# quadjr/aframe-gaussian-splatting

Hardware: AMD Instinct MI355X
Metric: frames/sec @1920x1080 (sort+project+bin+blend per frame, 1M-splat train.splat-shaped scene) (higher is better)
Workload: dtype f32

## Files before the change

### aframe-gaussian-splatting_amd/csrc/gs_prims.hip

```cpp
#include <type_traits>
#include "gs_internal.h"

namespace {

__device__ __forceinline__ uint32_t wave_incl_scan(uint32_t v, int lane)
{
#pragma unroll
    for (int d = 1; d < 64; d <<= 1) {
        const uint32_t t = __shfl_up(v, d, 64);
        if (lane >= d) v += t;
    }
    return v;
}

template <int NW>
__device__ __forceinline__ uint32_t block_excl_scan(uint32_t v, uint32_t *s_wave , uint32_t *total)
{
    const int lane = threadIdx.x & 63, w = threadIdx.x >> 6;
    const uint32_t inc = wave_incl_scan(v, lane);
    if (lane == 63) s_wave[w] = inc;
    __syncthreads();
    uint32_t base = 0, tot = 0;
#pragma unroll
    for (int k = 0; k < NW; k++) { const uint32_t s = s_wave[k]; if (k < w) base += s; tot += s; }
    __syncthreads();
    *total = tot;
    return base + inc - v;
}


template <bool PACKED, int NW>
__device__ __forceinline__ void k_radix_hist_body(const uint32_t *__restrict__ keys, const uint32_t *n_ptr, int shift,
                                                  int bits, uint32_t *__restrict__ hist)
{
    constexpr int NT = 64 * NW, IPT = 8, CH = NT * IPT;
    __shared__ uint32_t s_hist[GS_RADIX_MAX_BINS];
    const uint32_t n = *n_ptr;
    const uint32_t nchunks = (n + CH - 1) / CH;
    const uint32_t nbins = 1u << bits, mask = nbins - 1, rs = gs_radix_row_stride(nbins);
    for (uint32_t v = blockIdx.x; v < ((nchunks + 7u) & ~7u); v += gridDim.x) {
        uint32_t c;
        if (!gs_xcd_chunk(v, nchunks, c)) continue;
        for (uint32_t d = threadIdx.x; d < rs; d += NT) s_hist[d] = 0;
        __syncthreads();
        uint32_t kk[IPT];
#pragma unroll
        for (int r = 0; r < IPT; r++) {
            const uint32_t i = c * CH + r * NT + threadIdx.x;
            kk[r] = i < n ? keys[PACKED ? 2 * (size_t)i : i] : 0u;
        }
#pragma unroll
        for (int r = 0; r < IPT; r++) {
            const uint32_t i = c * CH + r * NT + threadIdx.x;
            if (i < n) atomicAdd(&s_hist[(kk[r] >> shift) & mask], 1u);
        }
        __syncthreads();
        for (uint32_t d = threadIdx.x; d < rs; d += NT) hist[(size_t)c * rs + d] = s_hist[d];
        __syncthreads();
    }
}

template <bool PACKED, int NW>
__global__ __launch_bounds__(64 * NW) void k_radix_hist(const uint32_t *__restrict__ keys, const uint32_t *n_ptr, int shift,
                                                        int bits, uint32_t *__restrict__ hist)
{
    k_radix_hist_body<PACKED, NW>(keys, n_ptr, shift, bits, hist);
}

template <int NW>
__device__ __forceinline__ void k_radix_scan_body(uint32_t *__restrict__ hist, const uint32_t *n_ptr, uint32_t chunk, int bits,
                                                  uint32_t *__restrict__ totals)
{
    constexpr int RC = 16;
    constexpr uint32_t LANES = 16u * NW;
    __shared__ uint4 s_part[NW][4];
    const uint32_t n = *n_ptr;
    const uint32_t nchunks = (n + chunk - 1) / chunk;
    const uint32_t nbins = 1u << bits, rs = gs_radix_row_stride(nbins);
    const uint32_t q = threadIdx.x & 3u, r = threadIdx.x >> 2;
    const int lane = threadIdx.x & 63, w = threadIdx.x >> 6;
    const uint32_t d0 = blockIdx.x * 16u + q * 4u;
    const bool dig_ok = d0 < rs;
    const uint32_t rpl = (nchunks + LANES - 1u) / LANES;
    const uint32_t c_lo = min(r * rpl, nchunks), c_hi = min(c_lo + rpl, nchunks);
    uint32_t *col = hist + d0;
    uint4 h[RC];
    uint4 run = make_uint4(0, 0, 0, 0);
#pragma unroll
    for (int k = 0; k < RC; k++) {
        h[k] = (dig_ok && c_lo + k < c_hi) ? *reinterpret_cast<const uint4 *>(col + (size_t)(c_lo + k) * rs) : make_uint4(0, 0, 0, 0);
    }
#pragma unroll
    for (int k = 0; k < RC; k++) { run.x += h[k].x; run.y += h[k].y; run.z += h[k].z; run.w += h[k].w; }
    if (dig_ok) {
        uint32_t c = c_lo + RC;
        for (; c + 8u <= c_hi; c += 8u) {
            uint4 t[8];
#pragma unroll
            for (int k = 0; k < 8; k++) t[k] = *reinterpret_cast<const uint4 *>(col + (size_t)(c + k) * rs);
#pragma unroll
            for (int k = 0; k < 8; k++) { run.x += t[k].x; run.y += t[k].y; run.z += t[k].z; run.w += t[k].w; }
        }
        for (; c < c_hi; c++) { const uint4 t = *reinterpret_cast<const uint4 *>(col + (size_t)c * rs); run.x += t.x; run.y += t.y; run.z += t.z; run.w += t.w; }
    }
    uint4 inc = run;
#pragma unroll
    for (int dlt = 4; dlt < 64; dlt <<= 1) {
        const uint32_t x = __shfl_up(inc.x, dlt, 64), y = __shfl_up(inc.y, dlt, 64), z = __shfl_up(inc.z, dlt, 64), ww = __shfl_up(inc.w, dlt, 64);
        if (lane >= dlt) { inc.x += x; inc.y += y; inc.z += z; inc.w += ww; }
    }
    if (lane >= 60) s_part[w][q] = inc;
    __syncthreads();
    uint4 base = make_uint4(inc.x - run.x, inc.y - run.y, inc.z - run.z, inc.w - run.w);
    uint4 grand = make_uint4(0, 0, 0, 0);
#pragma unroll
    for (int k = 0; k < NW; k++) {
        const uint4 p = s_part[k][q];
        if (k < w) { base.x += p.x; base.y += p.y; base.z += p.z; base.w += p.w; }
        grand.x += p.x; grand.y += p.y; grand.z += p.z; grand.w += p.w;
    }
    if (dig_ok) {
#pragma unroll
        for (int k = 0; k < RC; k++) {
            if (c_lo + k < c_hi) *reinterpret_cast<uint4 *>(col + (size_t)(c_lo + k) * rs) = base;
            base.x += h[k].x; base.y += h[k].y; base.z += h[k].z; base.w += h[k].w;
        }
        uint32_t c = c_lo + RC;
        for (; c + 8u <= c_hi; c += 8u) {
            uint4 t[8];
#pragma unroll
            for (int k = 0; k < 8; k++) t[k] = *reinterpret_cast<const uint4 *>(col + (size_t)(c + k) * rs);
#pragma unroll
            for (int k = 0; k < 8; k++) {
                *reinterpret_cast<uint4 *>(col + (size_t)(c + k) * rs) = base;
                base.x += t[k].x; base.y += t[k].y; base.z += t[k].z; base.w += t[k].w;
            }
        }
        for (; c < c_hi; c++) {
            const uint4 t = *reinterpret_cast<const uint4 *>(col + (size_t)c * rs);
            *reinterpret_cast<uint4 *>(col + (size_t)c * rs) = base;
            base.x += t.x; base.y += t.y; base.z += t.z; base.w += t.w;
        }
        if (r == 0) *reinterpret_cast<uint4 *>(totals + d0) = grand;
    }
}

template <int NW>
__global__ __launch_bounds__(64 * NW) void k_radix_scan(uint32_t *__restrict__ hist, const uint32_t *n_ptr, uint32_t chunk, int bits,
                                                        uint32_t *__restrict__ totals)
{
    k_radix_scan_body<NW>(hist, n_ptr, chunk, bits, totals);
}

template <int IN_FMT, int OUT_FMT, int MAXB, int NW>
__device__ __forceinline__ void k_radix_scatter_body(const void *__restrict__ in, void *__restrict__ out,
                                                     const uint32_t *n_ptr, int shift, int bits, uint32_t zero_key,
                                                     const uint32_t *__restrict__ hist_scanned, const uint32_t *__restrict__ totals,
                                                     int idx_bits, uint32_t *count_out, const uint32_t *fill_to)
{
    constexpr int NT = 64 * NW, IPT = 8, CH = NT * IPT;
    constexpr bool KEYONLY = (IN_FMT == GS_RADIX_KEYONLY && OUT_FMT == GS_RADIX_KEYONLY) || IN_FMT == GS_RADIX_KEYIDX;
    __shared__ uint32_t s_cnt[NW][MAXB];
    constexpr int MATCHB = MAXB <= 256 ? MAXB : 256;
    __shared__ unsigned long long s_match[NW][MATCHB];
    __shared__ uint32_t s_dbase[MAXB];
    __shared__ uint32_t s_gb[MAXB];
    __shared__ uint32_t s_k[CH];
    __shared__ uint32_t s_v[KEYONLY ? 1 : CH];
    __shared__ uint32_t s_wave[NW];
    const uint32_t n = *n_ptr;
    const uint32_t nchunks = (n + CH - 1) / CH;
    const uint32_t nbins = 1u << bits, mask = nbins - 1, rs = gs_radix_row_stride(nbins);
    const int lane = threadIdx.x & 63, w = threadIdx.x >> 6;
    const unsigned long long lt = (1ull << lane) - 1ull;
    if (IN_FMT == GS_RADIX_KEYIDX && fill_to) {
        const uint32_t upto = *fill_to;
        for (uint32_t i = n + blockIdx.x * NT + threadIdx.x; i < upto; i += gridDim.x * NT) reinterpret_cast<uint32_t *>(out)[i] = 0u;
    }
    if (blockIdx.x >= ((nchunks + 7u) & ~7u) && !(count_out && blockIdx.x == 0)) return;
    {
        constexpr int DPT = (MAXB + NT - 1) / NT;
        uint32_t tv[DPT], sum = 0;
#pragma unroll
        for (int k = 0; k < DPT; k++) { const uint32_t d = threadIdx.x * DPT + k; tv[k] = d < nbins ? totals[d] : 0u; sum += tv[k]; }
        uint32_t tot;
        uint32_t ex = block_excl_scan<NW>(sum, s_wave, &tot);
#pragma unroll
        for (int k = 0; k < DPT; k++) { const uint32_t d = threadIdx.x * DPT + k; if (d < nbins) s_dbase[d] = ex; ex += tv[k]; }
        if (count_out && blockIdx.x == 0 && threadIdx.x == 0) *count_out = tot;
    }
    for (uint32_t v = blockIdx.x; v < ((nchunks + 7u) & ~7u); v += gridDim.x) {
        uint32_t c;
        if (!gs_xcd_chunk(v, nchunks, c)) continue;
        for (uint32_t i = threadIdx.x; i < NW * MAXB; i += NT) { (&s_cnt[0][0])[i] = 0; if (i < NW * MATCHB) (&s_match[0][0])[i] = 0ull; }
        __syncthreads();
        uint32_t key[IPT], val[IPT], rank[IPT];
#pragma unroll
        for (int r = 0; r < IPT; r++) {
            const uint32_t i = c * CH + w * (CH / NW) + r * 64 + lane;
            const bool ok = i < n;
            if (IN_FMT == GS_RADIX_PACKED) {
                const uint2 kv = ok ? reinterpret_cast<const uint2 *>(in)[i] : make_uint2(0xFFFFFFFFu, 0u);
                key[r] = kv.x; val[r] = kv.y;
            } else {
                key[r] = ok ? reinterpret_cast<const uint32_t *>(in)[i] : 0xFFFFFFFFu;
                val[r] = i;
            }
        }
#pragma unroll
        for (int r = 0; r < IPT; r++) {
            const uint32_t i = c * CH + w * (CH / NW) + r * 64 + lane;
            bool ok = i < n;
            const uint32_t d = (key[r] >> shift) & mask;
            if (IN_FMT == GS_RADIX_KEYS) ok = ok && key[r] != GS_RADIX_SKIP;
            const uint32_t dm = d & (uint32_t)(MATCHB - 1);
            if (ok) atomicOr(&s_match[w][dm], 1ull << lane);
            __builtin_amdgcn_wave_barrier();
            unsigned long long peers = ok ? s_match[w][dm] : 0ull;
            if (MAXB > MATCHB) {
                const bool top = (d >> 8) & 1u;
                const unsigned long long vb = __ballot(ok && top);
                peers &= top ? vb : ~vb;
            }
            const uint32_t before = __popcll(peers & lt), cnt = __popcll(peers);
            const uint32_t prev = ok ? s_cnt[w][d] : 0u;
            __builtin_amdgcn_wave_barrier();
            if (ok && before == 0) { s_cnt[w][d] = prev + cnt; s_match[w][dm] = 0ull; }
            __builtin_amdgcn_wave_barrier();
            rank[r] = prev + before;
        }
        __syncthreads();
        uint32_t chunk_items;
        {
            constexpr int DPT = (MAXB + NT - 1) / NT;
            uint32_t tv[DPT], sum = 0;
#pragma unroll
            for (int k = 0; k < DPT; k++) {
                const uint32_t d = threadIdx.x * DPT + k;
                tv[k] = 0;
                if (d < nbins) {
#pragma unroll
                    for (int q = 0; q < NW; q++) tv[k] += s_cnt[q][d];
                }
                sum += tv[k];
            }
            uint32_t tot;
            uint32_t ex = block_excl_scan<NW>(sum, s_wave, &tot);
            chunk_items = tot;
#pragma unroll
            for (int k = 0; k < DPT; k++) {
                const uint32_t d = threadIdx.x * DPT + k;
                if (d < nbins) {
                    uint32_t run = ex;
#pragma unroll
                    for (int q = 0; q < NW; q++) { const uint32_t cq = s_cnt[q][d]; s_cnt[q][d] = run; run += cq; }
                    s_gb[d] = s_dbase[d] + hist_scanned[(size_t)c * rs + d] - ex;
                }
                ex += tv[k];
            }
        }
        __syncthreads();
#pragma unroll
        for (int r = 0; r < IPT; r++) {
            const uint32_t i = c * CH + w * (CH / NW) + r * 64 + lane;
            if (i < n && (IN_FMT != GS_RADIX_KEYS || key[r] != GS_RADIX_SKIP)) {
                const uint32_t d = (key[r] >> shift) & mask;
                s_k[s_cnt[w][d] + rank[r]] = key[r];
                if (!KEYONLY) s_v[s_cnt[w][d] + rank[r]] = val[r];
            }
        }
        __syncthreads();
        const uint32_t items = chunk_items;
#pragma unroll
        for (int r = 0; r < IPT; r++) {
            const uint32_t slot = r * NT + threadIdx.x;
            if (slot < items) {
                const uint2 kv = make_uint2(s_k[slot], KEYONLY ? 0u : s_v[slot]);
                const uint32_t pos = s_gb[(kv.x >> shift) & mask] + slot;
                if (OUT_FMT == GS_RADIX_PACKED) reinterpret_cast<uint2 *>(out)[pos] = kv;
                else if (OUT_FMT == GS_RADIX_KEYONLY) reinterpret_cast<uint32_t *>(out)[pos] = kv.x;
                else if (OUT_FMT == GS_RADIX_KEYIDX) reinterpret_cast<uint32_t *>(out)[pos] = ((kv.x >> (shift + bits)) << idx_bits) | kv.y;
                else if (IN_FMT == GS_RADIX_KEYIDX) reinterpret_cast<uint32_t *>(out)[pos] = kv.x & ((1u << shift) - 1u);
                else reinterpret_cast<uint32_t *>(out)[pos] = kv.x == zero_key ? 0u : kv.y;
            }
        }
        __syncthreads();
    }
}

template <int IN_FMT, int OUT_FMT, int MAXB, int NW>
__global__ __launch_bounds__(64 * NW) void k_radix_scatter(const void *__restrict__ in, void *__restrict__ out,
                                                           const uint32_t *n_ptr, int shift, int bits, uint32_t zero_key,
                                                           const uint32_t *__restrict__ hist_scanned, const uint32_t *__restrict__ totals,
                                                           int idx_bits, uint32_t *count_out, const uint32_t *fill_to)
{
    k_radix_scatter_body<IN_FMT, OUT_FMT, MAXB, NW>(in, out, n_ptr, shift, bits, zero_key, hist_scanned, totals, idx_bits, count_out, fill_to);
}

template <int BATCH>
__device__ __forceinline__ uint32_t msd_column_sum(const uint32_t *__restrict__ A, uint32_t na, const uint32_t *__restrict__ Bt, uint32_t b0, uint32_t b1, uint32_t dg)
{
    const uint32_t total = na + (b1 - b0);
    uint32_t sum = 0;
    for (uint32_t v0 = 0; v0 < total; v0 += (uint32_t)BATCH) {
        uint32_t t[BATCH];
#pragma unroll
        for (int k = 0; k < BATCH; k++) {
            const uint32_t v = v0 + (uint32_t)k < total ? v0 + (uint32_t)k : v0;
            const uint32_t *row = v < na ? A + (size_t)v * 256u : Bt + (size_t)(b0 + (v - na)) * 256u;
            t[k] = row[dg];
        }
#pragma unroll
        for (int k = 0; k < BATCH; k++) sum += v0 + (uint32_t)k < total ? t[k] : 0u;
    }
    return sum;
}

template <int IPT>
__device__ __forceinline__ void wave_digit_ranks(const uint32_t *dig, const bool *ok, unsigned long long *s_match, uint32_t *s_cnt, uint32_t *rank, int lane)
{
    const unsigned long long lt = (1ull << lane) - 1ull;
    uint32_t prev[IPT], before[IPT];
    int leader[IPT];
#pragma unroll
    for (int r = 0; r < IPT; r++) {
        if (ok[r]) atomicOr(&s_match[dig[r]], 1ull << lane);
        __builtin_amdgcn_wave_barrier();
        const unsigned long long peers = ok[r] ? s_match[dig[r]] : 0ull;
        before[r] = (uint32_t)__popcll(peers & lt);
        leader[r] = peers ? __ffsll((long long)peers) - 1 : 0;
        uint32_t pv = 0;
        if (ok[r] && before[r] == 0u) { pv = atomicAdd(&s_cnt[dig[r]], (uint32_t)__popcll(peers)); s_match[dig[r]] = 0ull; }
        __builtin_amdgcn_wave_barrier();
        prev[r] = pv;
    }
#pragma unroll
    for (int r = 0; r < IPT; r++) rank[r] = (uint32_t)__shfl((int)prev[r], leader[r], 64) + before[r];
}

#ifndef GS_SEG_B
#define GS_SEG_B 4096u
#endif
#define GS_SEG_MAXBLK 8u
template <int NW>
__device__ __forceinline__ void k_msd_scatter_body(const uint32_t *__restrict__ keys, uint32_t *__restrict__ rec, const uint32_t *n_ptr,
                                                   const uint32_t *__restrict__ rows, const uint32_t *__restrict__ grp, uint32_t *count_out,
                                                   uint32_t *__restrict__ seg_tab, uint32_t tail_req, GsControl *ctl, uint32_t n_host)
{
    constexpr int NT = 64 * NW, IPT = 8, CH = NT * IPT, NB = 256, PB = 24;
    __shared__ uint32_t s_cnt[NW][NB];
    __shared__ unsigned long long s_match[NW][NB];
    __shared__ uint32_t s_dbase[NB], s_gb[NB];
    __shared__ uint32_t s_k[CH], s_v[CH];
    __shared__ uint32_t s_wave[NW];
    __shared__ uint32_t s_cut, s_thr;
    const uint32_t n = n_host ? n_host : *n_ptr;
    const uint32_t nchunks = (n + CH - 1) / CH, ngroups = (nchunks + GS_MSD_GROUP - 1u) / GS_MSD_GROUP;
    const int lane = threadIdx.x & 63, w = threadIdx.x >> 6;
    const uint32_t dg = threadIdx.x < (uint32_t)NB ? threadIdx.x : 0u;
    const bool has_dg = threadIdx.x < (uint32_t)NB;
    const uint32_t vend = (nchunks + 7u) & ~7u;
    if (blockIdx.x >= vend && !(count_out && blockIdx.x == 0)) return;
    uint32_t key[IPT], pt[PB];
    uint32_t c = 0;
    auto load_chunk = [&](uint32_t cc) {
#pragma unroll
        for (int r = 0; r < IPT; r++) {
            const uint32_t i = cc * CH + w * (CH / NW) + r * 64 + lane;
            key[r] = keys[i < n ? i : n - 1u];
        }
        const uint32_t g0 = cc / GS_MSD_GROUP, nrow = g0 + (cc - g0 * GS_MSD_GROUP);
#pragma unroll
        for (int k = 0; k < PB; k++) {
            const uint32_t vv = (uint32_t)k < nrow ? (uint32_t)k : 0u;
            const uint32_t *row = (nrow == 0u || vv < g0) ? grp + (size_t)vv * 256u : rows + (size_t)(g0 * GS_MSD_GROUP + (vv - g0)) * 256u;
            pt[k] = row[dg];
        }
    };
    bool preloaded = blockIdx.x < vend && gs_xcd_chunk(blockIdx.x, nchunks, c);
    if (preloaded) load_chunk(c);
    for (uint32_t i = threadIdx.x; i < NW * NB; i += NT) (&s_match[0][0])[i] = 0ull;
    if (threadIdx.x == 0) { s_cut = 0u; s_thr = 0u; }
    uint32_t thr = 0u;
    {
        const uint32_t tot_d = has_dg ? msd_column_sum<16>(grp, ngroups, grp, 0u, 0u, dg) : 0u;
        uint32_t tot;
        uint32_t ex = block_excl_scan<NW>(tot_d, s_wave, &tot);
        if (tail_req && tail_req < tot) {
            const uint32_t suffix = tot - ex;
            if (has_dg && suffix >= tail_req && suffix - tot_d < tail_req) { s_cut = ex; s_thr = dg; }
            __syncthreads();
        }
        const uint32_t cut = s_cut;
        thr = s_thr;
        ex -= ex >= cut ? cut : ex;
        if (has_dg) s_dbase[dg] = ex;
        if (count_out && blockIdx.x == 0 && threadIdx.x == 0) *count_out = tot - cut;
        if (tail_req && blockIdx.x == 0 && threadIdx.x == 0) { ctl->near_sorted = 3u; ctl->n_valid = tot; }
        if (blockIdx.x == 0) {
            const uint32_t nbk = (tot_d && dg >= thr) ? (tot_d + GS_SEG_B - 1u) / GS_SEG_B : 0u;
            const uint32_t ni = nbk > GS_SEG_MAXBLK ? 1u : nbk;
            uint32_t nitems;
            const uint32_t ix = block_excl_scan<NW>(has_dg ? ni : 0u, s_wave, &nitems);
            uint4 *items = reinterpret_cast<uint4 *>(seg_tab + 4);
            if (has_dg) for (uint32_t j = 0; j < ni; j++) items[ix + j] = make_uint4(ex, tot_d, j, nbk > GS_SEG_MAXBLK ? 0xFFFFFFFFu : nbk);
            if (threadIdx.x == 0) { seg_tab[0] = nitems; seg_tab[1] = tot - cut; }
        }
    }
    for (uint32_t v = blockIdx.x; v < vend; v += gridDim.x) {
        if (!preloaded) { if (!gs_xcd_chunk(v, nchunks, c)) continue; load_chunk(c); }
        preloaded = false;
        for (uint32_t i = threadIdx.x; i < NW * NB; i += NT) (&s_cnt[0][0])[i] = 0;
        __syncthreads();
        uint32_t rank[IPT];
        const uint32_t g0 = c / GS_MSD_GROUP, nrow = g0 + (c - g0 * GS_MSD_GROUP);
        {
            uint32_t dig[IPT]; bool ok[IPT];
#pragma unroll
            for (int r = 0; r < IPT; r++) {
                if (c * CH + w * (CH / NW) + r * 64 + lane >= n) key[r] = GS_RADIX_SKIP;
                dig[r] = (key[r] >> 8) & 255u;
                if (dig[r] < thr) key[r] = GS_RADIX_SKIP;
                ok[r] = key[r] != GS_RADIX_SKIP;
            }
            wave_digit_ranks<IPT>(dig, ok, &s_match[w][0], &s_cnt[w][0], rank, lane);
        }
        uint32_t pre = 0;
#pragma unroll
        for (int k = 0; k < PB; k++) pre += (uint32_t)k < nrow ? pt[k] : 0u;
        for (uint32_t v0 = PB; v0 < nrow; v0 += 16u) {
            uint32_t t[16];
#pragma unroll
            for (int k = 0; k < 16; k++) {
                const uint32_t vv = v0 + (uint32_t)k < nrow ? v0 + (uint32_t)k : v0;
                const uint32_t *row = vv < g0 ? grp + (size_t)vv * 256u : rows + (size_t)(g0 * GS_MSD_GROUP + (vv - g0)) * 256u;
                t[k] = row[dg];
            }
#pragma unroll
            for (int k = 0; k < 16; k++) pre += v0 + (uint32_t)k < nrow ? t[k] : 0u;
        }
        __syncthreads();
        uint32_t chunk_items;
        {
            uint32_t tv = 0;
            if (has_dg) {
#pragma unroll
                for (int q = 0; q < NW; q++) tv += s_cnt[q][dg];
            }
            uint32_t tot;
            const uint32_t ex = block_excl_scan<NW>(tv, s_wave, &tot);
            chunk_items = tot;
            if (has_dg) {
                uint32_t run = ex;
#pragma unroll
                for (int q = 0; q < NW; q++) { const uint32_t cq = s_cnt[q][dg]; s_cnt[q][dg] = run; run += cq; }
                s_gb[dg] = s_dbase[dg] + pre - ex;
            }
        }
        __syncthreads();
#pragma unroll
        for (int r = 0; r < IPT; r++) {
            if (key[r] != GS_RADIX_SKIP) {
                const uint32_t d = (key[r] >> 8) & 255u;
                s_k[s_cnt[w][d] + rank[r]] = key[r];
                s_v[s_cnt[w][d] + rank[r]] = c * CH + w * (CH / NW) + r * 64 + lane;
            }
        }
        __syncthreads();
#pragma unroll
        for (int r = 0; r < IPT; r++) {
            const uint32_t slot = r * NT + threadIdx.x;
            if (slot < chunk_items) {
                const uint32_t k = s_k[slot];
                rec[s_gb[(k >> 8) & 255u] + slot] = ((k & 255u) << 24) | s_v[slot];
            }
        }
        __syncthreads();
    }
}

template <int NW, int R>
__device__ __forceinline__ void seg_sort_block(const uint32_t *__restrict__ blk, uint32_t items, uint32_t *__restrict__ out, uint32_t (*s_cnt)[256],
                                               unsigned long long (*s_match)[256], const uint32_t *s_dbase, uint32_t *s_cur, uint32_t *s_gb, uint32_t *s_k,
                                               uint32_t *s_wave, uint32_t start, bool multi)
{
    constexpr int NT = 64 * NW, NB = 256;
    const int lane = threadIdx.x & 63, w = threadIdx.x >> 6;
    const uint32_t dg = threadIdx.x < (uint32_t)NB ? threadIdx.x : 0u;
    const bool has_dg = threadIdx.x < (uint32_t)NB;
    for (uint32_t i = threadIdx.x; i < NW * NB; i += NT) (&s_cnt[0][0])[i] = 0;
    __syncthreads();
    uint32_t key[R];
#pragma unroll
    for (int r = 0; r < R; r++) {
        key[r] = blk[w * (R * 64) + r * 64 + lane];
    }
#pragma unroll
    for (int r = 0; r < R; r++)
        if ((uint32_t)(w * (R * 64) + r * 64 + lane) < items) atomicAdd(&s_cnt[w][key[r] >> 24], 1u);
    __syncthreads();
    {
        uint32_t tv = 0;
        if (has_dg) {
#pragma unroll
            for (int q = 0; q < NW; q++) tv += s_cnt[q][dg];
        }
        uint32_t tot;
        const uint32_t ex = block_excl_scan<NW>(tv, s_wave, &tot);
        if (has_dg) {
            uint32_t run = ex;
#pragma unroll
            for (int q = 0; q < NW; q++) { const uint32_t cq = s_cnt[q][dg]; s_cnt[q][dg] = run; run += cq; }
            s_gb[dg] = multi ? start + s_dbase[dg] + s_cur[dg] - ex : start;
            if (multi) s_cur[dg] += tv;
        }
    }
    __syncthreads();
#pragma unroll
    for (int h = 0; h < R / 8; h++) {
        uint32_t dig[8], slot[8]; bool ok[8];
#pragma unroll
        for (int r = 0; r < 8; r++) { ok[r] = (uint32_t)(w * (R * 64) + (h * 8 + r) * 64 + lane) < items; dig[r] = key[h * 8 + r] >> 24; }
        wave_digit_ranks<8>(dig, ok, &s_match[w][0], &s_cnt[w][0], slot, lane);
#pragma unroll
        for (int r = 0; r < 8; r++) if (ok[r]) s_k[slot[r]] = key[h * 8 + r];
    }
    __syncthreads();
#pragma unroll 8
    for (int r = 0; r < R; r++) {
        const uint32_t slot = r * NT + threadIdx.x;
        if (slot < items) { const uint32_t k = s_k[slot]; out[s_gb[k >> 24] + slot] = k & 0x00FFFFFFu; }
    }
    __syncthreads();
}

template <int NW, int IPT>
__device__ __forceinline__ void k_seg_sort_body(const uint32_t *__restrict__ rec, uint32_t *__restrict__ out, const uint32_t *__restrict__ seg_tab, const uint32_t *fill_to)
{
    constexpr int NT = 64 * NW, B = NT * IPT, NB = 256;
    static_assert(NT >= NB && IPT == 16 && B == (int)GS_SEG_B, "one digit per thread; blocks of 8 / 16 rounds");
    __shared__ uint32_t s_cnt[NW][NB];
    __shared__ unsigned long long s_match[NW][NB];
    __shared__ uint32_t s_dbase[NB], s_cur[NB], s_gb[NB];
    __shared__ uint32_t s_k[B];
    __shared__ uint32_t s_wave[NW];
    const uint32_t dg = threadIdx.x < (uint32_t)NB ? threadIdx.x : 0u;
    const bool has_dg = threadIdx.x < (uint32_t)NB;
    const uint4 *items = reinterpret_cast<const uint4 *>(seg_tab + 4);
    const uint4 first_item = items[blockIdx.x];
    const uint32_t nitems = seg_tab[0], total = seg_tab[1];
    for (uint32_t i = threadIdx.x; i < NW * NB; i += NT) (&s_match[0][0])[i] = 0ull;
    if (fill_to) {
        const uint32_t upto = *fill_to;
        for (uint32_t i = total + blockIdx.x * NT + threadIdx.x; i < upto; i += gridDim.x * NT) out[i] = 0u;
    }
    for (uint32_t v = blockIdx.x; v < nitems; v += gridDim.x) {
        const uint4 it = v == blockIdx.x ? first_item : items[v];
        const uint32_t start = it.x, len = it.y, blk = it.z, nblk = it.w;
        const uint32_t *seg = rec + start;
        __syncthreads();
        if (nblk == 1u) {
            if (len <= (uint32_t)NT * 8u) seg_sort_block<NW, 8>(seg, len, out, s_cnt, s_match, s_dbase, s_cur, s_gb, s_k, s_wave, start, false);
            else seg_sort_block<NW, 16>(seg, len, out, s_cnt, s_match, s_dbase, s_cur, s_gb, s_k, s_wave, start, false);
            continue;
        }
        const bool all = nblk == 0xFFFFFFFFu;
        const uint32_t before = all ? 0u : blk * (uint32_t)B;
        if (has_dg) { s_cur[dg] = 0; s_dbase[dg] = 0; }
        __syncthreads();
        for (uint32_t i0 = 0; i0 < len; i0 += 16u * NT) {
            uint32_t t[16];
#pragma unroll
            for (int k = 0; k < 16; k++) t[k] = seg[i0 + (uint32_t)k * NT + threadIdx.x];
#pragma unroll
            for (int k = 0; k < 16; k++) {
                const uint32_t i = i0 + (uint32_t)k * NT + threadIdx.x;
                if (i < len) { atomicAdd(&s_dbase[t[k] >> 24], 1u); if (i < before) atomicAdd(&s_cur[t[k] >> 24], 1u); }
            }
        }
        __syncthreads();
        const uint32_t tv = has_dg ? s_dbase[dg] : 0u;
        uint32_t tt;
        const uint32_t ex = block_excl_scan<NW>(tv, s_wave, &tt);
        if (has_dg) s_dbase[dg] = ex;
        __syncthreads();
        if (!all) {
            const uint32_t items_b = len - before < (uint32_t)B ? len - before : (uint32_t)B;
            seg_sort_block<NW, 16>(seg + before, items_b, out, s_cnt, s_match, s_dbase, s_cur, s_gb, s_k, s_wave, start, true);
        } else {
            for (uint32_t b = 0; b * (uint32_t)B < len; b++) {
                const uint32_t items_b = len - b * (uint32_t)B < (uint32_t)B ? len - b * (uint32_t)B : (uint32_t)B;
                seg_sort_block<NW, 16>(seg + (size_t)b * B, items_b, out, s_cnt, s_match, s_dbase, s_cur, s_gb, s_k, s_wave, start, true);
            }
        }
    }
}

template <int NW>
__global__ __launch_bounds__(64 * NW, 4) void k_msd_scatter(const uint32_t *__restrict__ keys, uint32_t *__restrict__ rec, const uint32_t *n_ptr,
                                                         const uint32_t *__restrict__ rows, const uint32_t *__restrict__ grp, uint32_t *count_out,
                                                         uint32_t *__restrict__ seg_tab, uint32_t tail_req, GsControl *ctl, uint32_t n_host)
{
    k_msd_scatter_body<NW>(keys, rec, n_ptr, rows, grp, count_out, seg_tab, tail_req, ctl, n_host);
}
template <int NW, int IPT>
__global__ __launch_bounds__(64 * NW, 4) void k_seg_sort(const uint32_t *__restrict__ rec, uint32_t *__restrict__ out, const uint32_t *__restrict__ seg_tab, const uint32_t *fill_to)
{
    k_seg_sort_body<NW, IPT>(rec, out, seg_tab, fill_to);
}
template <int NW> GS_BODY(F_msd_scatter, (k_msd_scatter<NW>), (k_msd_scatter_body<NW>));
template <int NW, int IPT> GS_BODY(F_seg_sort, (k_seg_sort<NW, IPT>), (k_seg_sort_body<NW, IPT>));
#define GS_SEG_GRID 512u
#ifndef GS_SEG_NW
#define GS_SEG_NW 4
#endif
#ifndef GS_SEG_IPT
#define GS_SEG_IPT 16
#endif

uint32_t grid_for(uint32_t items, uint32_t chunk)
{
    uint32_t g = gs_div_up(items, chunk);
    if (g < 1) g = 1;
    const uint32_t cap = chunk == GS_CHUNK_L ? 1024u : 2048u;
    if (g > cap) g = cap;
    return (g + 7u) & ~7u;
}

template <bool PACKED, int NW> GS_BODY(F_hist, (k_radix_hist<PACKED, NW>), (k_radix_hist_body<PACKED, NW>));
template <int NW> GS_BODY(F_scan, (k_radix_scan<NW>), (k_radix_scan_body<NW>));
template <int I, int O, int B, int NW> GS_BODY(F_scatter, (k_radix_scatter<I, O, B, NW>), (k_radix_scatter_body<I, O, B, NW>));

template <int NW, int NF>
int launch_pass(gs_ctx *const S[], const GsRadixIO io[], int in_fmt, int out_fmt, uint32_t hint_n, int shift, int bits, bool have_hist, uint32_t zero_key, int idx_bits)
{
    constexpr uint32_t CH = 64 * NW * 8;
    constexpr int NT = 64 * NW;
    gs_ctx *ctx = S[0];
    const uint32_t g = grid_for(hint_n, CH);
    hipStream_t st = ctx->stream;
    if (!have_hist) {
        const auto args = [&](int k) { return gs_pack_make((const uint32_t *)io[k].in, io[k].n_ptr, shift, bits, S[k]->hist); };
        if (in_fmt == GS_RADIX_PACKED) gs_launch<NF, F_hist<true, NW>, NT>(g, st, 0, args);
        else gs_launch<NF, F_hist<false, NW>, NT>(g, st, 0, args);
    }
    gs_launch<NF, F_scan<NW>, NT>(gs_div_up(gs_radix_row_stride(1u << bits), 16u), st, 0,
                                  [&](int k) { return gs_pack_make(S[k]->hist, io[k].n_ptr, CH, bits, S[k]->radix_aux); });
    const auto scatter = [&](auto I, auto O) {
        const auto args = [&](int k) { return gs_pack_make(io[k].in, io[k].out, io[k].n_ptr, shift, bits, zero_key, (const uint32_t *)S[k]->hist,
                                                           (const uint32_t *)S[k]->radix_aux, idx_bits, io[k].count_out, io[k].fill_to); };
        if (bits <= 7) gs_launch<NF, F_scatter<decltype(I)::value, decltype(O)::value, 128, NW>, NT>(g, st, 0, args);
        else if (bits == 8) gs_launch<NF, F_scatter<decltype(I)::value, decltype(O)::value, 256, NW>, NT>(g, st, 0, args);
        else gs_launch<NF, F_scatter<decltype(I)::value, decltype(O)::value, GS_RADIX_MAX_BINS, NW>, NT>(g, st, 0, args);
    };
    typedef std::integral_constant<int, GS_RADIX_KEYS> Keys;
    typedef std::integral_constant<int, GS_RADIX_PACKED> Packed;
    typedef std::integral_constant<int, GS_RADIX_KEYIDX> KeyIdx;
    bool known = true;
    if (in_fmt == GS_RADIX_PACKED && out_fmt == GS_RADIX_PACKED) scatter(Packed(), Packed());
    else if (in_fmt == GS_RADIX_PACKED && out_fmt == GS_RADIX_KEYS) scatter(Packed(), Keys());
    else if (in_fmt == GS_RADIX_PACKED && out_fmt == GS_RADIX_KEYIDX) scatter(Packed(), KeyIdx());
    else if (in_fmt == GS_RADIX_KEYS && out_fmt == GS_RADIX_PACKED) scatter(Keys(), Packed());
    else if (in_fmt == GS_RADIX_KEYS && out_fmt == GS_RADIX_KEYIDX) scatter(Keys(), KeyIdx());
    else if (in_fmt == GS_RADIX_KEYIDX && out_fmt == GS_RADIX_KEYS) scatter(KeyIdx(), Keys());
    else if (in_fmt == GS_RADIX_KEYS && out_fmt == GS_RADIX_KEYS) {
        if constexpr (NF == 1) scatter(Keys(), Keys()); else known = false;
    } else known = false;
    if (!known) { snprintf(GS_ERRBUF(ctx), GS_ERRLEN, "radix pass: unsupported record formats %d -> %d", in_fmt, out_fmt); return GS_E_BADARG; }
    GS_HIP(hipGetLastError());
    return GS_OK;
}

}

template <int NF>
int gs_radix_pass(gs_ctx *const S[], const GsRadixIO io[], int in_fmt, int out_fmt, uint32_t max_n, uint32_t hint_n, int shift, int bits, bool have_hist,
                  uint32_t zero_key, int idx_bits)
{
    gs_ctx *ctx = S[0];
    if (bits < 1 || bits > 9) { snprintf(GS_ERRBUF(ctx), GS_ERRLEN, "radix pass: %d-bit digit (1..9 supported)", bits); return GS_E_BADARG; }
    if (hint_n > max_n || hint_n == 0) hint_n = max_n;
    return gs_radix_chunk(hint_n) == GS_CHUNK_L ? launch_pass<8, NF>(S, io, in_fmt, out_fmt, hint_n, shift, bits, have_hist, zero_key, idx_bits)
                                                : launch_pass<4, NF>(S, io, in_fmt, out_fmt, hint_n, shift, bits, have_hist, zero_key, idx_bits);
}
template int gs_radix_pass<1>(gs_ctx *const[], const GsRadixIO[], int, int, uint32_t, uint32_t, int, int, bool, uint32_t, int);
template int gs_radix_pass<2>(gs_ctx *const[], const GsRadixIO[], int, int, uint32_t, uint32_t, int, int, bool, uint32_t, int);

template <int NF>
int gs_msd_sort(gs_ctx *const S[], uint32_t n, const uint32_t tail_req[])
{
    gs_ctx *ctx = S[0];
    for (int k = 0; k < NF; k++)
        if ((size_t)S[k]->scratch_cap * 2 < (size_t)n + GS_SEG_B) { snprintf(GS_ERRBUF(ctx), GS_ERRLEN, "msd sort: scratch of %zu splats is too small for %u records", S[k]->scratch_cap, n); return GS_E_STATE; }
    const uint32_t chunk = gs_radix_chunk(n), g = grid_for(n, chunk);
    hipStream_t st = ctx->stream;
    const auto scatter = [&](int k) { return gs_pack_make((const uint32_t *)S[k]->key_a, reinterpret_cast<uint32_t *>(S[k]->kv_b), (const uint32_t *)&S[k]->ctl->n_total, (const uint32_t *)S[k]->hist,
                                                          (const uint32_t *)S[k]->msd_grp, &S[k]->ctl->n_sorted, S[k]->msd_tab, tail_req[k], S[k]->ctl, n); };
    if (chunk == GS_CHUNK_L) gs_launch<NF, F_msd_scatter<8>, 512, 4>(g, st, 0, scatter);
    else gs_launch<NF, F_msd_scatter<4>, 256, 4>(g, st, 0, scatter);
    gs_launch<NF, F_seg_sort<GS_SEG_NW, GS_SEG_IPT>, 64 * GS_SEG_NW, 4>(GS_SEG_GRID, st, 0, [&](int k) {
        return gs_pack_make((const uint32_t *)reinterpret_cast<uint32_t *>(S[k]->kv_b), S[k]->val_a, (const uint32_t *)S[k]->msd_tab,
                            tail_req[k] ? (const uint32_t *)nullptr : (const uint32_t *)&S[k]->ctl->n_kept); });
    GS_HIP(hipGetLastError());
    return GS_OK;
}
template int gs_msd_sort<1>(gs_ctx *const[], uint32_t, const uint32_t[]);
template int gs_msd_sort<2>(gs_ctx *const[], uint32_t, const uint32_t[]);

uint32_t gs_radix_chunk(uint32_t hint_n) { return hint_n > GS_RADIX_LARGE_N ? GS_CHUNK_L : GS_CHUNK_S; }
uint32_t gs_radix_grid(uint32_t hint_n) { return grid_for(hint_n, gs_radix_chunk(hint_n)); }
```

Measured before the change: 20670.

## Compact surviving keys before ranking in tail-cut radix scatter pass

```diff
diff --git a/aframe-gaussian-splatting_amd/csrc/gs_prims.hip b/aframe-gaussian-splatting_amd/csrc/gs_prims.hip
--- a/aframe-gaussian-splatting_amd/csrc/gs_prims.hip
+++ b/aframe-gaussian-splatting_amd/csrc/gs_prims.hip
@@ -382,10 +382,12 @@
     for (uint32_t i = threadIdx.x; i < NW * NB; i += NT) (&s_match[0][0])[i] = 0ull;
     if (threadIdx.x == 0) { s_cut = 0u; s_thr = 0u; }
     uint32_t thr = 0u;
+    bool cut_on = false;
     {
         const uint32_t tot_d = has_dg ? msd_column_sum<16>(grp, ngroups, grp, 0u, 0u, dg) : 0u;
         uint32_t tot;
         uint32_t ex = block_excl_scan<NW>(tot_d, s_wave, &tot);
+        cut_on = tail_req && tail_req < tot;
         if (tail_req && tail_req < tot) {
             const uint32_t suffix = tot - ex;
             if (has_dg && suffix >= tail_req && suffix - tot_d < tail_req) { s_cut = ex; s_thr = dg; }
@@ -411,33 +413,85 @@
         if (!preloaded) { if (!gs_xcd_chunk(v, nchunks, c)) continue; load_chunk(c); }
         preloaded = false;
         for (uint32_t i = threadIdx.x; i < NW * NB; i += NT) (&s_cnt[0][0])[i] = 0;
-        __syncthreads();
         uint32_t rank[IPT];
         const uint32_t g0 = c / GS_MSD_GROUP, nrow = g0 + (c - g0 * GS_MSD_GROUP);
+        const auto chunk_pre = [&]() {
+            uint32_t pre = 0;
+#pragma unroll
+            for (int k = 0; k < PB; k++) pre += (uint32_t)k < nrow ? pt[k] : 0u;
+            for (uint32_t v0 = PB; v0 < nrow; v0 += 16u) {
+                uint32_t t[16];
+#pragma unroll
+                for (int k = 0; k < 16; k++) {
+                    const uint32_t vv = v0 + (uint32_t)k < nrow ? v0 + (uint32_t)k : v0;
+                    const uint32_t *row = vv < g0 ? grp + (size_t)vv * 256u : rows + (size_t)(g0 * GS_MSD_GROUP + (vv - g0)) * 256u;
+                    t[k] = row[dg];
+                }
+#pragma unroll
+                for (int k = 0; k < 16; k++) pre += v0 + (uint32_t)k < nrow ? t[k] : 0u;
+            }
+            return pre;
+        };
+#pragma unroll
+        for (int r = 0; r < IPT; r++) {
+            if (c * CH + w * (CH / NW) + r * 64 + lane >= n) key[r] = GS_RADIX_SKIP;
+            if (((key[r] >> 8) & 255u) < thr) key[r] = GS_RADIX_SKIP;
+        }
+        constexpr uint32_t CAP = NT;
+        if (cut_on) {
+            uint32_t wcnt = 0;
+#pragma unroll
+            for (int r = 0; r < IPT; r++) wcnt += (uint32_t)__popcll(__ballot(key[r] != GS_RADIX_SKIP));
+            if (lane == 0) s_wave[w] = wcnt;
+        }
+        __syncthreads();
+        uint32_t s_c = CAP + 1u, wbase = 0;
+        if (cut_on) {
+            s_c = 0;
+#pragma unroll
+            for (int q = 0; q < NW; q++) { const uint32_t t = s_wave[q]; if (q < w) wbase += t; s_c += t; }
+            if (s_c == 0u) { __syncthreads(); continue; }
+        }
+        const uint32_t pre = chunk_pre();
+        {
+            if (s_c <= CAP) {
+                if (has_dg) s_gb[dg] = s_dbase[dg] + pre;
+                const unsigned long long lt = (1ull << lane) - 1ull;
+                uint32_t at = wbase;
+#pragma unroll
+                for (int r = 0; r < IPT; r++) {
+                    const bool ok = key[r] != GS_RADIX_SKIP;
+                    const unsigned long long bal = __ballot(ok);
+                    if (ok) {
+                        const uint32_t p = at + (uint32_t)__popcll(bal & lt);
+                        s_k[p] = key[r];
+                        s_v[p] = c * CH + w * (CH / NW) + r * 64 + lane;
+                    }
+                    at += (uint32_t)__popcll(bal);
+                }
+                __syncthreads();
+                const bool mine = threadIdx.x < s_c;
+                uint32_t k1 = 0, d1 = 0, r1 = 0;
+                if ((uint32_t)w * 64u < s_c) {
+                    if (mine) k1 = s_k[threadIdx.x];
+                    d1 = (k1 >> 8) & 255u;
+                    wave_digit_ranks<1>(&d1, &mine, &s_match[w][0], &s_cnt[w][0], &r1, lane);
+                }
+                __syncthreads();
+                if (mine) {
+#pragma unroll
+                    for (int q = 0; q < NW - 1; q++) if (q < w) r1 += s_cnt[q][d1];
+                    rec[s_gb[d1] + r1] = ((k1 & 255u) << 24) | s_v[threadIdx.x];
+                }
+                __syncthreads();
+                continue;
+            }
+        }
         {
             uint32_t dig[IPT]; bool ok[IPT];
 #pragma unroll
-            for (int r = 0; r < IPT; r++) {
-                if (c * CH + w * (CH / NW) + r * 64 + lane >= n) key[r] = GS_RADIX_SKIP;
-                dig[r] = (key[r] >> 8) & 255u;
-                if (dig[r] < thr) key[r] = GS_RADIX_SKIP;
-                ok[r] = key[r] != GS_RADIX_SKIP;
-            }
+            for (int r = 0; r < IPT; r++) { dig[r] = (key[r] >> 8) & 255u; ok[r] = key[r] != GS_RADIX_SKIP; }
             wave_digit_ranks<IPT>(dig, ok, &s_match[w][0], &s_cnt[w][0], rank, lane);
-        }
-        uint32_t pre = 0;
-#pragma unroll
-        for (int k = 0; k < PB; k++) pre += (uint32_t)k < nrow ? pt[k] : 0u;
-        for (uint32_t v0 = PB; v0 < nrow; v0 += 16u) {
-            uint32_t t[16];
-#pragma unroll
-            for (int k = 0; k < 16; k++) {
-                const uint32_t vv = v0 + (uint32_t)k < nrow ? v0 + (uint32_t)k : v0;
-                const uint32_t *row = vv < g0 ? grp + (size_t)vv * 256u : rows + (size_t)(g0 * GS_MSD_GROUP + (vv - g0)) * 256u;
-                t[k] = row[dg];
-            }
-#pragma unroll
-            for (int k = 0; k < 16; k++) pre += v0 + (uint32_t)k < nrow ? t[k] : 0u;
         }
         __syncthreads();
         uint32_t chunk_items;
```

Result: faster. 20940, median of 6 (+1.3%).
